# antao97/SegGroup

Hardware: AMD Instinct MI355X
Metric: pseudo-label scenes/sec (150k pts, 1.5k segs) (higher is better)
Workload: dtype f32 (fp32 accumulate; operands split into 2 x fp16 pieces on v_mfma_f32_32x32x16_f16; kNN / FPS scores in exact fp32 order); 1 GPU; 64 distinct synthetic scenes per GPU per step, 150000 pts / 1500 segs each (BASELINE.json configs[2]; configs[1] = the same scene shape, single scene); mode=ins_infer, scenes_in_flight=112, engine=14 groups x 8 scenes per batched launch, weights=tests/golden/weights_g2.npz, parallelism=scene-parallel x1

## Files before the change

### include/seggroup_hip.h

```cpp
#ifndef SEGGROUP_HIP_H
#define SEGGROUP_HIP_H

#include <stddef.h>
#include <stdint.h>

#ifdef __cplusplus
extern "C" {
#endif

#define SG_OK          0
#define SG_EINVAL     -1
#define SG_EHIP       -2
#define SG_ENOMEM     -3
#define SG_ESTALL     -4
#define SG_EUNSUP     -5
#define SG_EINTERNAL  -6

#define SG_MODE_INS_INFER 0
#define SG_MODE_SEM_INFER 1

#define SG_NUM_LABEL_VECTORS 14
#define SG_RANGE_WORDS 256
#define SG_MAX_POINTS (1 << 20)

const char* sg_last_error(void);
int  sg_version(void);
int  sg_device_count(void);
int  sg_selftest_wave_ops(int* h_mismatches, void* stream);
int  sg_selftest_list_insert(int* h_mismatches, void* stream);

size_t sg_contract_ws_bytes(int S);
int sg_contract_point_edges(const int64_t* d_adj, int E, const int32_t* d_seg_of_point, int N, int S,
                            int32_t* d_out_adj, int out_capacity, int32_t* d_out_count,
                            void* d_ws, size_t ws_bytes, void* stream);

int sg_gather_members(const int32_t* d_seg_points, const int32_t* d_seg_off, int S,
                      const int32_t* d_order, const int32_t* d_dst, const int32_t* d_cl,
                      int32_t* d_members, int32_t* d_pos_of_point, int32_t* d_cluster_of_pos,
                      int32_t* d_slot_of_pos, void* stream);

size_t sg_fps_ws_bytes(int N);
int sg_fps_sample(const float* d_data, int N, int ch_in, const int32_t* d_members, const int32_t* d_cl_off, int C,
                  int P, int ch_out, int transform, float* d_samples, int32_t* d_sel,
                  void* d_ws, size_t ws_bytes, void* stream);

size_t sg_mlp1_ws_bytes(int C);
int sg_mlp1_forward(const float* d_samples, int C, const float* d_w, const float* d_gamma, const float* d_beta,
                    float* d_feat, int feat_stride, void* d_ws, size_t ws_bytes, void* stream);

int sg_edge_distance(const float* d_feat, int feat_stride, int D, const int32_t* d_adj, int E,
                     float* d_dist, void* stream);

int sg_group_max_rows(const float* d_rows, int row_stride, int D, const int32_t* d_goff, const int32_t* d_gidx,
                      int G, float* d_out, int out_stride, void* stream);

int sg_segment_max(const float* d_rows, int N, int D, const int32_t* d_cluster_of_pos,
                   float* d_out, int out_stride, int C, void* stream);

size_t sg_center_ws_bytes(int T, int C);
int sg_center_clusters(const float* d_data, int N, const int32_t* d_members, const int32_t* d_cl_off, int C,
                       const int32_t* d_tile_cl, const int32_t* d_tile_lo, const int32_t* d_tile_hi, int T,
                       const int32_t* d_cl_tile_off, float* d_x9m, float* d_xyzw,
                       void* d_ws, size_t ws_bytes, void* stream);

int sg_cluster_knn(const float* d_xyzw, int N, const int32_t* d_cl_off,
                   const int32_t* d_tile_cl, const int32_t* d_tile_lo, const int32_t* d_tile_hi, int T,
                   int k, int pos0, int32_t* d_knn, void* stream);

int sg_segment_boxes(const float* d_data, const int32_t* d_seg_points, const int32_t* d_seg_off, int S,
                     float* d_box, void* stream);
int sg_cluster_knn_pruned(const float* d_xyzw, int N, const int32_t* d_cl_off,
                          const int32_t* d_tile_cl, const int32_t* d_tile_lo, const int32_t* d_tile_hi, int T,
                          const int32_t* d_cl_seg_off, const int32_t* d_order, const int32_t* d_dst,
                          const int32_t* d_seg_off, const float* d_segbox, const int32_t* d_slot_of_pos,
                          int k, int pos0, int32_t* d_knn, void* stream);

size_t sg_segment_sort_ws_bytes(int N);
int sg_segment_sort_boxes(const float* d_data, int N, const int32_t* d_seg_points, const int32_t* d_seg_off,
                          const int32_t* d_seg_of_point, int S, const int32_t* d_seg_chunk_off, int max_seg, float* d_segbox,
                          int32_t* d_sperm, float* d_chunk_box, double* d_seg_sums, void* d_ws, size_t ws_bytes, void* stream);
int sg_layer_layout(const float* d_data, int N, const int32_t* d_seg_points, const int32_t* d_seg_off, const int32_t* d_sperm, int S,
                    const int32_t* d_order, const int32_t* d_dst, const int32_t* d_cl, const float* d_cl_mean, int32_t* d_members,
                    int32_t* d_pos_of_point, int32_t* d_cluster_of_pos, int32_t* d_slot_of_pos, float* d_x9m, float* d_sxyzw,
                    int32_t* d_smpos, float* d_point_rec, int32_t* d_seed_id, unsigned int* d_range_bits, void* stream);
int sg_knn_operands(const float* d_data, const int32_t* d_seg_points, const int32_t* d_seg_off, const int32_t* d_sperm, int S,
                    const int32_t* d_order, const int32_t* d_dst, float* d_sxyzw, int32_t* d_smpos, void* stream);
int sg_cluster_knn_sorted(const float* d_sxyzw, const int32_t* d_smpos, int N, const int32_t* d_cl_off,
                          const int32_t* d_tile_cl, const int32_t* d_tile_lo, const int32_t* d_tile_hi, int T,
                          const int32_t* d_cl_seg_off, const int32_t* d_order, const int32_t* d_dst,
                          const int32_t* d_seg_off, const int32_t* d_seg_chunk_off, const float* d_segbox,
                          const float* d_chunk_box, const int32_t* d_slot_of_pos, int k, int pos0, int32_t* d_knn, void* stream);
int sg_knn_seed_points(const int32_t* d_knn, const int32_t* d_members, int N, int k, int32_t* d_seed, void* stream);
int sg_cluster_knn_seeded(const float* d_sxyzw, const int32_t* d_smpos, int N, const int32_t* d_cl_off,
                          const int32_t* d_tile_cl, const int32_t* d_tile_lo, const int32_t* d_tile_hi, int T,
                          const int32_t* d_cl_seg_off, const int32_t* d_order, const int32_t* d_dst,
                          const int32_t* d_seg_off, const int32_t* d_seg_chunk_off, const float* d_segbox,
                          const float* d_chunk_box, const int32_t* d_slot_of_pos, const int32_t* d_seed,
                          const int32_t* d_seg_prevcl, const int32_t* d_members, const float* d_point_rec,
                          int k, int pos0, int32_t* d_knn, void* stream);

int sg_knn_chunk_table(const int32_t* d_order, const int32_t* d_dst, const int32_t* d_seg_off, const int32_t* d_seg_chunk_off,
                       const float* d_chunk_box, int S, const int32_t* d_slot_chunk0, float* d_cc, void* stream);
int sg_cluster_knn_2pass(const float* d_sxyzw, const int32_t* d_smpos, int N, const int32_t* d_cl_off,
                         const int32_t* d_tile_cl, const int32_t* d_tile_lo, const int32_t* d_tile_hi,
                         const int32_t* d_tile_chunk0, int T, const int32_t* d_cl_chunk_off, const float* d_cc,
                         int k, int pos0, int32_t* d_knn, void* stream);
int sg_cluster_knn_sorted_w(const float* d_sxyzw, const int32_t* d_smpos, int N, const int32_t* d_cl_off,
                            const int32_t* d_tile_cl, const int32_t* d_tile_lo, const int32_t* d_tile_hi, int T,
                            const int32_t* d_cl_seg_off, const int32_t* d_order, const int32_t* d_dst,
                            const int32_t* d_seg_off, const int32_t* d_seg_chunk_off, const float* d_segbox,
                            const float* d_chunk_box, const int32_t* d_slot_of_pos, int k, int pos0, int waves_per_tile,
                            int32_t* d_knn, void* stream);

size_t sg_edgeconv_ws_bytes(int N);
int sg_edgeconv_forward(const float* d_x9m, const int32_t* d_knn, int N, int k, int layers,
                        const float* d_w1, const float* d_g1, const float* d_b1,
                        const float* d_w2, const float* d_g2, const float* d_b2,
                        float* d_out, void* d_ws, size_t ws_bytes, void* stream);
int sg_edgeconv_forward_r(const float* d_x9m, const int32_t* d_knn, int N, int k, int layers, const float* d_w1, const float* d_g1,
                          const float* d_b1, const float* d_w2, const float* d_g2, const float* d_b2, float* d_out, void* d_ws,
                          size_t ws_bytes, unsigned int* d_range_bits, void* stream);
#define SG_EDGECONV_COMPILER_LOOP 1u
int sg_edgeconv_forward_x(const float* d_x9m, const int32_t* d_knn, int N, int k, int layers, const float* d_w1, const float* d_g1,
                          const float* d_b1, const float* d_w2, const float* d_g2, const float* d_b2, float* d_out, void* d_ws,
                          size_t ws_bytes, unsigned int* d_range_bits, unsigned int flags, void* stream);
int sg_edge_range(const float* d_x9m, int N, unsigned int* d_range_bits, void* stream);

size_t sg_gcn_ws_bytes(int S, int D, int E);
int sg_gcn_forward(const float* d_x, int S, int D, const int32_t* d_adj, int E,
                   const int32_t* d_rowptr, const int32_t* d_col, const int32_t* d_eid,
                   const float* d_w, float alpha, float* d_out, void* d_ws, size_t ws_bytes, void* stream);

int sg_export_labels(const int32_t* d_unmap, int V, const int32_t* d_seg_of_point, int N,
                     const int32_t* d_tables, int T, int S, int32_t* d_out, void* stream);

size_t sg_eval_ws_bytes(int max_ins);
int sg_evaluate(const int32_t* d_gt, const int32_t* d_sem_pred, const int32_t* d_ins_pred, int V, int max_ins,
                float* h_iou_sem, float* h_iou_ins, float* h_acc, void* d_ws, size_t ws_bytes, void* stream);

typedef struct sg_partition sg_partition;

sg_partition* sg_partition_create(int S, const int32_t* h_seg_first, const int32_t* h_seg_size,
                                  const int32_t* h_seg_ins, const int32_t* h_seg_sem);
void sg_partition_destroy(sg_partition* p);
int  sg_partition_num_clusters(const sg_partition* p);

int sg_partition_union(sg_partition* p, int seg_root1, int seg_root2);
int sg_partition_find(const sg_partition* p, int s);
int sg_partition_label(const sg_partition* p, int r, int32_t* ins, int32_t* sem, double* npts);

int sg_partition_layer(const sg_partition* p, int32_t* h_root, int32_t* h_cl_of_seg, int32_t* h_order,
                       int32_t* h_cl_seg_off, int32_t* h_cl_pt_off, int32_t* h_dst);

int sg_partition_group_nearby(sg_partition* p, const int32_t* h_root, int C, const float* h_dist,
                              const int32_t* h_adj, int E, float th, uint8_t* h_connected);

int sg_partition_contract(const sg_partition* p, const int32_t* h_root_old, const int32_t* h_adj, int E,
                          const uint8_t* h_keep, int32_t* h_adj_out);

int sg_partition_group_unlabeled(sg_partition* p, int32_t* h_root_io, int* C_io, float* h_feat, int D,
                                 int32_t* h_adj, int* E_io);
int sg_partition_unlabeled_fallback(sg_partition* p, const int32_t* h_root, int C, const float* h_samples, int P);

int sg_partition_export_tables(const sg_partition* p, int32_t* h_seg_tab, int32_t* h_ins_tab, int32_t* h_sem_tab);

typedef struct sg_pipeline sg_pipeline;

typedef struct sg_weights {
    const float* mlp1_w;  const float* mlp1_g;  const float* mlp1_b;
    const float* mlp2_w;  const float* mlp2_g;  const float* mlp2_b;
    const float* gcn2_w;
    const float* mlp3_w1; const float* mlp3_g1; const float* mlp3_b1;
    const float* mlp3_w2; const float* mlp3_g2; const float* mlp3_b2;
    const float* gcn3_w;
} sg_weights;

typedef struct sg_scene {
    int N, S, E0, V;
    const float*   d_data;
    const int64_t* d_adj;
    const int32_t* d_seg_of_point;
    const int32_t* d_seg_points;
    const int32_t* d_seg_off;
    const int32_t* d_unmap;
    const int32_t* d_gt;
    const int32_t* h_seg_first;
    const int32_t* h_seg_size;
    const int32_t* h_seg_ins;
    const int32_t* h_seg_sem;
    const int32_t* h_seg_of_vertex;
} sg_scene;

typedef struct sg_result {
    int32_t* h_labels;
    float iou_sem[80];
    float iou_ins[80];
    float acc[4];
    int32_t trace[5];
    int32_t stalled;
    int32_t used_fallback;
    int32_t* h_tables;
// ... 425 lines not shown
```

### seggroup_amd/csrc/kernels_mlp1.hip

```cpp
#include "engine_ctx.h"
#include "sg_common.h"
#include "knn_device.h"
#include "wave_ops.h"

namespace {

constexpr int K1 = 10;

__device__ inline float knn_score(float xq, float yq, float zq, float xxq, float xc, float yc, float zc, float xxc) {
    const float t = __builtin_fmaf(zq, zc, __builtin_fmaf(yq, yc, xq * xc));
    const float inner = -2.0f * t;
    return ((-xxc) - inner) - xxq;
}

__device__ inline float sqnorm3(float x, float y, float z) { return (x * x + y * y) + z * z; }

__device__ __forceinline__ void mlp1_knn_moments_body(const float* __restrict__ samples, uint8_t* __restrict__ knn,
                                                      double* __restrict__ partial, int c) {
    const int lane = threadIdx.x;
    const float* row = samples + ((size_t)c * 64 + lane) * 6;
    float f[6];
#pragma unroll
    for (int k = 0; k < 6; ++k) f[k] = row[k];
    const float xx = sqnorm3(f[0], f[1], f[2]);

    double kvl[K1];
#pragma unroll
    for (int t = 0; t < K1; ++t) kvl[t] = sgknn::list_empty();
#pragma unroll 8
    for (int j = 0; j < 64; ++j) {
        const float s = knn_score(f[0], f[1], f[2], xx, sgw::bcast(f[0], j), sgw::bcast(f[1], j), sgw::bcast(f[2], j), sgw::bcast(xx, j));
        sgknn::list_insert<K1>(kvl, sgknn::make_key(s, j));
    }
    int bi[K1];
#pragma unroll
    for (int t = 0; t < K1; ++t) bi[t] = sgknn::list_index(kvl[t]);
    uint8_t* ko = knn + ((size_t)c * 64 + lane) * K1;
#pragma unroll
    for (int t = 0; t < K1; ++t) ko[t] = (uint8_t)bi[t];

    double e[K1][6];
    double m0 = 0, m1 = 0, m2 = 0;
#pragma unroll
    for (int t = 0; t < K1; ++t) {
#pragma unroll
        for (int k = 0; k < 6; ++k) e[t][k] = (double)__shfl(f[k], bi[t]);
        m0 += e[t][0]; m1 += e[t][1]; m2 += e[t][2];
    }
    m0 /= K1; m1 /= K1; m2 /= K1;
    double acc[27];
#pragma unroll
    for (int q = 0; q < 27; ++q) acc[q] = 0.0;
#pragma unroll
    for (int t = 0; t < K1; ++t) {
        e[t][0] = (e[t][0] - m0) * 10.0; e[t][1] = (e[t][1] - m1) * 10.0; e[t][2] = (e[t][2] - m2) * 10.0;
        int q = 6;
#pragma unroll
        for (int a = 0; a < 6; ++a) {
            acc[a] += e[t][a];
#pragma unroll
            for (int b = a; b < 6; ++b) acc[q++] += e[t][a] * e[t][b];
        }
    }
#pragma unroll
    for (int q = 0; q < 27; ++q) {
        const double v = sgw::wave_sum(acc[q]);
        if (lane == 0) partial[(size_t)c * 27 + q] = v;
    }
}
__global__ __launch_bounds__(64) void k_mlp1_knn_moments(const float* __restrict__ samples, uint8_t* __restrict__ knn,
                                                         double* __restrict__ partial) {
    mlp1_knn_moments_body(samples, knn, partial, blockIdx.x);
}
__global__ __launch_bounds__(64) void k_mlp1_knn_moments_b(const sg::SlotCtx* __restrict__ cx) {
    const sg::SlotCtx& c = cx[blockIdx.y];
    if ((int)blockIdx.x >= c.S) return;
    mlp1_knn_moments_body(c.samples, c.m1_knn, c.m1_partial, blockIdx.x);
}

__device__ __forceinline__ void mlp1_finalize_body(const double* __restrict__ partial, int C, const float* __restrict__ w,
                                                   const float* __restrict__ gamma, const float* __restrict__ beta,
                                                   float* __restrict__ folded) {
    __shared__ double mom[27];
    {
        const int q = threadIdx.x >> 5, l = threadIdx.x & 31;
        double s = 0.0;
        for (int c = l; c < C; c += 32) s += partial[(size_t)c * 27 + q];
#pragma unroll
        for (int o = 16; o > 0; o >>= 1) s += __shfl_xor(s, o);
        if (l == 0) mom[q] = s / ((double)C * 64.0 * K1);
    }
    __syncthreads();
    const int ch = threadIdx.x;
    if (ch >= 64) return;
    double cov[6][6];
    int q = 6;
    for (int a = 0; a < 6; ++a)
        for (int b = a; b < 6; ++b) { cov[a][b] = cov[b][a] = mom[q] - mom[a] * mom[b]; ++q; }
    double mean = 0.0, var = 0.0;
    for (int a = 0; a < 6; ++a) {
        mean += (double)w[ch * 6 + a] * mom[a];
        for (int b = 0; b < 6; ++b) var += (double)w[ch * 6 + a] * (double)w[ch * 6 + b] * cov[a][b];
    }
    const double a_ = (double)gamma[ch] / sqrt(var + 1e-5);
    for (int k = 0; k < 6; ++k) folded[ch * 6 + k] = (float)(a_ * (double)w[ch * 6 + k]);
    folded[384 + ch] = (float)((double)beta[ch] - a_ * mean);
}
__global__ __launch_bounds__(27 * 32) void k_mlp1_finalize(const double* __restrict__ partial, int C, const float* __restrict__ w,
                                                           const float* __restrict__ gamma, const float* __restrict__ beta,
                                                           float* __restrict__ folded) {
    mlp1_finalize_body(partial, C, w, gamma, beta, folded);
}
__global__ __launch_bounds__(27 * 32) void k_mlp1_finalize_b(const sg::SlotCtx* __restrict__ cx, const float* __restrict__ w,
                                                             const float* __restrict__ gamma, const float* __restrict__ beta) {
    const sg::SlotCtx& c = cx[blockIdx.y];
    mlp1_finalize_body(c.m1_partial, c.S, w, gamma, beta, c.m1_folded);
}

__device__ __forceinline__ void mlp1_apply_body(const float* __restrict__ samples, const uint8_t* __restrict__ knn,
                                                const float* __restrict__ folded, float* __restrict__ feat, int feat_stride, int c) {
    const int lane = threadIdx.x;
    const float* row = samples + ((size_t)c * 64 + lane) * 6;
    float f[6];
#pragma unroll
    for (int k = 0; k < 6; ++k) f[k] = row[k];
    const uint8_t* ki = knn + ((size_t)c * 64 + lane) * K1;
    float e[K1][6];
    double m0 = 0, m1 = 0, m2 = 0;
    double ed[K1][3];
#pragma unroll
    for (int t = 0; t < K1; ++t) {
        const int j = ki[t];
#pragma unroll
        for (int k = 0; k < 6; ++k) e[t][k] = __shfl(f[k], j);
        ed[t][0] = e[t][0]; ed[t][1] = e[t][1]; ed[t][2] = e[t][2];
        m0 += ed[t][0]; m1 += ed[t][1]; m2 += ed[t][2];
    }
    m0 /= K1; m1 /= K1; m2 /= K1;
#pragma unroll
    for (int t = 0; t < K1; ++t) {
        e[t][0] = (float)((ed[t][0] - m0) * 10.0); e[t][1] = (float)((ed[t][1] - m1) * 10.0); e[t][2] = (float)((ed[t][2] - m2) * 10.0);
    }
    float* out = feat + (size_t)c * feat_stride;
    __shared__ float hs[64 * 65];
    __shared__ __attribute__((aligned(8))) float wl[448];
#pragma unroll
    for (int i = 0; i < 7; ++i) {
        const int e_ = lane + 64 * i;
        wl[e_ < 384 ? (e_ % 6) * 64 + e_ / 6 : e_] = folded[e_];
    }
    __builtin_amdgcn_wave_barrier();
    using f32x2 = __attribute__((ext_vector_type(2))) float;
#pragma unroll 2
    for (int ch = 0; ch < 64; ch += 2) {
        f32x2 w[6];
#pragma unroll
        for (int k = 0; k < 6; ++k) w[k] = *reinterpret_cast<const f32x2*>(&wl[k * 64 + ch]);
        const f32x2 b = *reinterpret_cast<const f32x2*>(&wl[384 + ch]);
        float h0 = -INFINITY, h1 = -INFINITY;
#pragma unroll
        for (int t = 0; t < K1; ++t) {
            f32x2 y = b;
#pragma unroll
            for (int k = 0; k < 6; ++k) y = __builtin_elementwise_fma(w[k], f32x2{e[t][k], e[t][k]}, y);
            h0 = fmaxf(h0, y.x);
            h1 = fmaxf(h1, y.y);
        }
        hs[ch * 65 + lane] = fmaxf(h0, 0.2f * h0);
        hs[(ch + 1) * 65 + lane] = fmaxf(h1, 0.2f * h1);
    }
    __builtin_amdgcn_wave_barrier();
    {
        const float* row = hs + lane * 65;
        float mx = -INFINITY;
        double sm = 0.0;
#pragma unroll 8
        for (int i = 0; i < 64; ++i) {
            const float v = row[i];
            mx = fmaxf(mx, v);
            sm += (double)v;
        }
        out[lane] = mx;
        out[64 + lane] = (float)(sm / 64.0);
    }
}
__global__ __launch_bounds__(64) void k_mlp1_apply(const float* __restrict__ samples, const uint8_t* __restrict__ knn,
                                                   const float* __restrict__ folded, float* __restrict__ feat, int feat_stride) {
    mlp1_apply_body(samples, knn, folded, feat, feat_stride, blockIdx.x);
}
__global__ __launch_bounds__(64) void k_mlp1_apply_b(const sg::SlotCtx* __restrict__ cx) {
    const sg::SlotCtx& c = cx[blockIdx.y];
    if ((int)blockIdx.x >= c.S) return;
    mlp1_apply_body(c.samples, c.m1_knn, c.m1_folded, c.feat1, 128, blockIdx.x);
}

__global__ __launch_bounds__(27 * 32) void k_mlp1_bwd_stats(const double* __restrict__ partial, int C, const float* __restrict__ w,
                                                            double* __restrict__ mom_out, float* __restrict__ cst, float* __restrict__ stats_out) {
    __shared__ double mom[27];
    {
        const int q = threadIdx.x >> 5, l = threadIdx.x & 31;
        double s = 0.0;
        for (int c = l; c < C; c += 32) s += partial[(size_t)c * 27 + q];
#pragma unroll
        for (int o = 16; o > 0; o >>= 1) s += __shfl_xor(s, o);
        if (l == 0) { mom[q] = s / ((double)C * 64.0 * K1); mom_out[q] = mom[q]; }
    }
    __syncthreads();
    const int ch = threadIdx.x;
    if (ch >= 64) return;
    double cov[6][6];
    int q = 6;
    for (int a = 0; a < 6; ++a)
        for (int b = a; b < 6; ++b) { cov[a][b] = cov[b][a] = mom[q] - mom[a] * mom[b]; ++q; }
    double mean = 0.0, var = 0.0;
    for (int a = 0; a < 6; ++a) {
        mean += (double)w[ch * 6 + a] * mom[a];
        for (int b = 0; b < 6; ++b) var += (double)w[ch * 6 + a] * (double)w[ch * 6 + b] * cov[a][b];
    }
    var = fmax(var, 0.0);
    cst[ch] = (float)mean;
    cst[64 + ch] = (float)(1.0 / sqrt(var + 1e-5));
    if (stats_out) { stats_out[ch] = (float)mean; stats_out[64 + ch] = (float)var; }
}

__global__ __launch_bounds__(64) void k_mlp1_bwd_rows(const float* __restrict__ samples, const uint8_t* __restrict__ knn, const float* __restrict__ w,
                                                      const float* __restrict__ gamma, const float* __restrict__ beta, const float* __restrict__ cst,
                                                      const float* __restrict__ gfeat, int g_stride, double* __restrict__ rows_partial) {
    const int c = blockIdx.x, lane = threadIdx.x;
    const float* row = samples + ((size_t)c * 64 + lane) * 6;
    float f[6];
#pragma unroll
    for (int k = 0; k < 6; ++k) f[k] = row[k];
    const uint8_t* ki = knn + ((size_t)c * 64 + lane) * K1;
    float e[K1][6];
    double m0 = 0, m1 = 0, m2 = 0;
    double ed[K1][3];
#pragma unroll
    for (int t = 0; t < K1; ++t) {
        const int j = ki[t];
#pragma unroll
        for (int k = 0; k < 6; ++k) e[t][k] = __shfl(f[k], j);
        ed[t][0] = e[t][0]; ed[t][1] = e[t][1]; ed[t][2] = e[t][2];
        m0 += ed[t][0]; m1 += ed[t][1]; m2 += ed[t][2];
    }
    m0 /= K1; m1 /= K1; m2 /= K1;
#pragma unroll
    for (int t = 0; t < K1; ++t) {
        e[t][0] = (float)((ed[t][0] - m0) * 10.0); e[t][1] = (float)((ed[t][1] - m1) * 10.0); e[t][2] = (float)((ed[t][2] - m2) * 10.0);
    }
    const float* g = gfeat + (size_t)c * g_stride;
    double* out = rows_partial + (size_t)c * 512;
    for (int ch = 0; ch < 64; ++ch) {
        const float w0 = w[ch * 6 + 0], w1 = w[ch * 6 + 1], w2 = w[ch * 6 + 2], w3 = w[ch * 6 + 3], w4 = w[ch * 6 + 4], w5 = w[ch * 6 + 5];
        const float mu = cst[ch], inv = cst[64 + ch], ga = gamma[ch], be = beta[ch];
        float best = -INFINITY, bx = 0.f, ba = 0.f;
        float be_[6] = {0.f, 0.f, 0.f, 0.f, 0.f, 0.f};
#pragma unroll
        for (int t = 0; t < K1; ++t) {
            float y = w0 * e[t][0];
            y = __builtin_fmaf(w1, e[t][1], y); y = __builtin_fmaf(w2, e[t][2], y);
            y = __builtin_fmaf(w3, e[t][3], y); y = __builtin_fmaf(w4, e[t][4], y); y = __builtin_fmaf(w5, e[t][5], y);
            const float xh = (y - mu) * inv;
            const float a = xh * ga + be;
            const float h = fmaxf(a, 0.2f * a);
            if (h > best) {
                best = h; bx = xh; ba = a;
#pragma unroll
                for (int k = 0; k < 6; ++k) be_[k] = e[t][k];
            }
        }
        float mv = best;
        int mi = lane;
        sgw::wave_argmax(mv, mi);
        const float dh = (lane == mi ? g[ch] : 0.f) + g[64 + ch] * (1.0f / 64.0f);
        const double da = (double)(dh * (ba > 0.f ? 1.f : 0.2f));
        const double v[8] = {da, da * (double)bx, da * (double)be_[0], da * (double)be_[1], da * (double)be_[2], da * (double)be_[3],
                             da * (double)be_[4], da * (double)be_[5]};
#pragma unroll
        for (int q = 0; q < 8; ++q) {
            const double r = sgw::wave_sum(v[q]);
            if (lane == 0) out[ch * 8 + q] = r;
        }
    }
}

__global__ __launch_bounds__(512) void k_mlp1_bwd_fold(const double* __restrict__ rows_partial, int nparts, int C, const double* __restrict__ mom,
                                                       const float* __restrict__ w, const float* __restrict__ gamma, const float* __restrict__ cst,
                                                       float* __restrict__ gw, float* __restrict__ gg, float* __restrict__ gb) {
    __shared__ double acc[512];
    const int t = threadIdx.x;
    double a = 0.0;
    for (int c = 0; c < nparts; ++c) a += rows_partial[(size_t)c * 512 + t];
    acc[t] = a;
    __syncthreads();
    const double rows = (double)C * 64.0 * K1;
    if (t < 64) { gb[t] = (float)acc[t * 8]; gg[t] = (float)acc[t * 8 + 1]; }
    if (t < 384) {
        const int ch = t / 6, j = t - ch * 6;
        const double inv = (double)cst[64 + ch], mu = (double)cst[ch];
        auto m2 = [&](int p, int q_) {
            const int lo = p < q_ ? p : q_, hi = p < q_ ? q_ : p;
            return mom[6 + lo * 6 - lo * (lo - 1) / 2 + (hi - lo)];
        };
        double wsee = 0.0;
        for (int q_ = 0; q_ < 6; ++q_) wsee += (double)w[ch * 6 + q_] * m2(q_, j);
        const double xe = (wsee - mu * mom[j]) * inv * rows;
        gw[t] = (float)((double)gamma[ch] * inv * (acc[ch * 8 + 2 + j] - acc[ch * 8] / rows * (mom[j] * rows) - acc[ch * 8 + 1] / rows * xe));
    }
}

}

namespace sg {

int b_mlp1(const SlotCtx* d_ctx, const float* d_w, const float* d_g, const float* d_b, const BatchDims& bd, hipStream_t st) {
    if (bd.nslots == 0 || bd.max_S == 0) return SG_OK;
    k_mlp1_knn_moments_b<<<dim3(bd.max_S, bd.nslots), 64, 0, st>>>(d_ctx);
    k_mlp1_finalize_b<<<dim3(1, bd.nslots), 27 * 32, 0, st>>>(d_ctx, d_w, d_g, d_b);
    k_mlp1_apply_b<<<dim3(bd.max_S, bd.nslots), 64, 0, st>>>(d_ctx);
    SG_LAUNCH_CHECK();
    return SG_OK;
}

}

extern "C" {

size_t sg_mlp1_ws_bytes(int C) {
    const size_t c = (size_t)std::max(C, 1);
    return sg::align_up(c * 64 * K1) + sg::align_up(c * 27 * 8) + sg::align_up(448 * 4);
}

int sg_mlp1_forward(const float* d_samples, int C, const float* d_w, const float* d_gamma, const float* d_beta, float* d_feat,
                    int feat_stride, void* d_ws, size_t ws_bytes, void* stream) {
    SG_REQUIRE(C >= 0 && feat_stride >= 128 && d_ws, "sg_mlp1_forward: bad arguments");
    if (C == 0) return SG_OK;
    sg::Carver cv(d_ws, ws_bytes);
    uint8_t* knn = cv.take<uint8_t>((size_t)C * 64 * K1);
    double* partial = cv.take<double>((size_t)C * 27);
    float* folded = cv.take<float>(448);
    if (!cv.ok) return sg::fail(SG_ENOMEM, "sg_mlp1_forward: workspace too small (%zu < %zu)", ws_bytes, sg_mlp1_ws_bytes(C));
    hipStream_t st = sg::as_stream(stream);
    k_mlp1_knn_moments<<<C, 64, 0, st>>>(d_samples, knn, partial);
    k_mlp1_finalize<<<1, 27 * 32, 0, st>>>(partial, C, d_w, d_gamma, d_beta, folded);
    k_mlp1_apply<<<C, 64, 0, st>>>(d_samples, knn, folded, d_feat, feat_stride);
    SG_LAUNCH_CHECK();
    return SG_OK;
}

size_t sg_mlp1_backward_ws_bytes(int C) {
    const size_t c = (size_t)std::max(C, 1);
    return sg::align_up(c * 64 * K1) + sg::align_up(c * 27 * 8) + sg::align_up(c * 512 * 8) + sg::align_up(27 * 8) + sg::align_up(128 * 4) + sg::align_up(512 * 8);
}

int sg_mlp1_backward(const float* d_samples, int C, const float* d_w, const float* d_gamma, const float* d_beta, const float* d_gfeat,
                     int g_stride, float* d_gw, float* d_gg, float* d_gb, float* d_bn_stats, void* d_ws, size_t ws_bytes, void* stream) {
    SG_REQUIRE(C > 0 && g_stride >= 128 && d_samples && d_w && d_gamma && d_beta && d_gfeat && d_gw && d_gg && d_gb && d_ws, "sg_mlp1_backward: bad arguments");
    sg::Carver cv(d_ws, ws_bytes);
    uint8_t* knn = cv.take<uint8_t>((size_t)C * 64 * K1);
    double* partial = cv.take<double>((size_t)C * 27);
    double* rows_partial = cv.take<double>((size_t)C * 512);
    double* mom = cv.take<double>(27);
    float* cst = cv.take<float>(128);
    double* red = cv.take<double>(512);
    if (!cv.ok) return sg::fail(SG_ENOMEM, "sg_mlp1_backward: workspace too small (%zu < %zu)", ws_bytes, sg_mlp1_backward_ws_bytes(C));
    hipStream_t st = sg::as_stream(stream);
    k_mlp1_knn_moments<<<C, 64, 0, st>>>(d_samples, knn, partial);
    k_mlp1_bwd_stats<<<1, 27 * 32, 0, st>>>(partial, C, d_w, mom, cst, d_bn_stats);
    k_mlp1_bwd_rows<<<C, 64, 0, st>>>(d_samples, knn, d_w, d_gamma, d_beta, cst, d_gfeat, g_stride, rows_partial);
    if (int rc = sg::reduce_partials(rows_partial, C, 512, 512, red, st)) return rc;
    k_mlp1_bwd_fold<<<1, 512, 0, st>>>(red, 1, C, mom, d_w, d_gamma, cst, d_gw, d_gg, d_gb);
    SG_LAUNCH_CHECK();
    return SG_OK;
}

}
```

### seggroup_amd/hip.py

```python
from __future__ import annotations

import contextlib
import ctypes as C
import os
import struct
import types
from typing import Optional

_HERE = os.path.dirname(os.path.abspath(__file__))
LIB_PATH = os.environ.get("SEGGROUP_HIP_LIB") or os.path.join(_HERE, "libseggroup_hip.so")
HOST_LIB_OVERRIDE = os.environ.get("SEGGROUP_HIP_HOST_LIB")

SG_OK, SG_EINVAL, SG_EHIP, SG_ENOMEM, SG_ESTALL, SG_EUNSUP, SG_EINTERNAL = 0, -1, -2, -3, -4, -5, -6
MODE_INS_INFER, MODE_SEM_INFER = 0, 1
COLOUR_SEMANTIC, COLOUR_INSTANCE, COLOUR_SEGMENT, COLOUR_GROUPING = 0, 1, 2, 3
NUM_LABEL_VECTORS = 14
KNN_BRUTE, KNN_GRID = 0, 1
KNN_INDEX = {"brute": KNN_BRUTE, "grid": KNN_GRID}
MAX_GRID_POINTS = 1 << 24
MAX_POINTS = 1 << 20
MAX_CLOUD_POINTS = 1 << 27
MAX_RADIUS_PAIRS = 1 << 30


def knn_index(index) -> int:
    if not isinstance(index, str) or index not in KNN_INDEX:
        raise ValueError("index must be 'brute' or 'grid', not %r" % (index,))
    return KNN_INDEX[index]


def knn_cell(cell) -> float:
    c = 0.0 if cell is None else float(cell)
    if not (c >= 0.0) or c == float("inf"):
        raise ValueError("cell must be a finite edge > 0, or None for the library's choice")
    return c
LABEL_NAMES = [f"layer_{l}.{k}" for l in (1, 2, 3, 4) for k in ("seg", "ins", "sem")] + ["final.ins", "final.sem"]

c_f32p = C.POINTER(C.c_float)
c_i32p = C.POINTER(C.c_int32)
c_i64p = C.POINTER(C.c_int64)
c_u8p = C.POINTER(C.c_uint8)
vp = C.c_void_p


class SgError(RuntimeError):
    def __init__(self, code: int, msg: str):
        super().__init__(f"libseggroup_hip error {code}: {msg}")
        self.code = code


class Weights(C.Structure):
    _fields_ = [(n, vp) for n in ("mlp1_w", "mlp1_g", "mlp1_b", "mlp2_w", "mlp2_g", "mlp2_b", "gcn2_w",
                                  "mlp3_w1", "mlp3_g1", "mlp3_b1", "mlp3_w2", "mlp3_g2", "mlp3_b2", "gcn3_w")]


class Scene(C.Structure):
    _fields_ = [("N", C.c_int), ("S", C.c_int), ("E0", C.c_int), ("V", C.c_int),
                ("d_data", vp), ("d_adj", vp), ("d_seg_of_point", vp), ("d_seg_points", vp), ("d_seg_off", vp),
                ("d_unmap", vp), ("d_gt", vp),
                ("h_seg_first", vp), ("h_seg_size", vp), ("h_seg_ins", vp), ("h_seg_sem", vp), ("h_seg_of_vertex", vp)]


class Result(C.Structure):
    _fields_ = [("h_labels", vp), ("iou_sem", C.c_float * 80), ("iou_ins", C.c_float * 80), ("acc", C.c_float * 4),
                ("trace", C.c_int32 * 5), ("stalled", C.c_int32), ("used_fallback", C.c_int32), ("h_tables", vp)]


class Classifier(C.Structure):
    _fields_ = [(n, vp) for n in ("w1", "gamma", "beta", "w2", "b2")]


class Debug(C.Structure):
    _fields_ = [("d_samples1", vp), ("d_feat1", vp), ("d_pointfeat", vp * 2), ("d_knn", vp * 2), ("d_members", vp * 2),
                ("h_gcn", vp * 2), ("h_dist", vp * 3), ("h_adj", vp * 4), ("n_adj", C.c_int32 * 4),
                ("h_feat5", vp), ("h_ins5", vp), ("h_sem5", vp), ("n5", C.c_int32), ("tape", vp), ("d_cat", vp * 2)]


_I, _Z = C.c_int, C.c_size_t
SIGNATURES = {
    "sg_last_error": (C.c_char_p, []),
    "sg_version": (_I, []),
    "sg_device_count": (_I, []),
    "sg_selftest_wave_ops": (_I, [C.POINTER(C.c_int), vp]),
    "sg_selftest_list_insert": (_I, [C.POINTER(C.c_int), vp]),
    "sg_contract_ws_bytes": (_Z, [_I]),
    "sg_contract_point_edges": (_I, [vp, _I, vp, _I, _I, vp, _I, vp, vp, _Z, vp]),
    "sg_gather_members": (_I, [vp, vp, _I, vp, vp, vp, vp, vp, vp, vp, vp]),
    "sg_fps_ws_bytes": (_Z, [_I]),
    "sg_fps_sample": (_I, [vp, _I, _I, vp, vp, _I, _I, _I, _I, vp, vp, vp, _Z, vp]),
    "sg_mlp1_ws_bytes": (_Z, [_I]),
    "sg_mlp1_forward": (_I, [vp, _I, vp, vp, vp, vp, _I, vp, _Z, vp]),
    "sg_edge_distance": (_I, [vp, _I, _I, vp, _I, vp, vp]),
    "sg_group_max_rows": (_I, [vp, _I, _I, vp, vp, _I, vp, _I, vp]),
    "sg_segment_max": (_I, [vp, _I, _I, vp, vp, _I, _I, vp]),
    "sg_center_ws_bytes": (_Z, [_I, _I]),
    "sg_center_clusters": (_I, [vp, _I, vp, vp, _I, vp, vp, vp, _I, vp, vp, vp, vp, _Z, vp]),
    "sg_cluster_knn": (_I, [vp, _I, vp, vp, vp, vp, _I, _I, _I, vp, vp]),
    "sg_segment_boxes": (_I, [vp, vp, vp, _I, vp, vp]),
    "sg_cluster_knn_pruned": (_I, [vp, _I, vp, vp, vp, vp, _I, vp, vp, vp, vp, vp, vp, _I, _I, vp, vp]),
    "sg_segment_sort_ws_bytes": (_Z, [_I]),
    "sg_knn_operands": (_I, [vp, vp, vp, vp, _I, vp, vp, vp, vp, vp]),
    "sg_cluster_knn_sorted": (_I, [vp, vp, _I, vp, vp, vp, vp, _I, vp, vp, vp, vp, vp, vp, vp, vp, _I, _I, vp, vp]),
    "sg_segment_sort_boxes": (_I, [vp, _I, vp, vp, vp, _I, vp, _I, vp, vp, vp, vp, vp, _Z, vp]),
    "sg_layer_layout": (_I, [vp, _I, vp, vp, vp, _I, vp, vp, vp, vp, vp, vp, vp, vp, vp, vp, vp, vp, vp, vp, vp]),
    "sg_cluster_knn_sorted_w": (_I, [vp, vp, _I, vp, vp, vp, vp, _I, vp, vp, vp, vp, vp, vp, vp, vp, _I, _I, _I, vp, vp]),
    "sg_knn_seed_points": (_I, [vp, vp, _I, _I, vp, vp]),
    "sg_cluster_knn_seeded": (_I, [vp, vp, _I, vp, vp, vp, vp, _I, vp, vp, vp, vp, vp, vp, vp, vp, vp, vp, vp, vp, _I, _I, vp, vp]),
    "sg_knn_chunk_table": (_I, [vp, vp, vp, vp, vp, _I, vp, vp, vp]),
    "sg_cluster_knn_2pass": (_I, [vp, vp, _I, vp, vp, vp, vp, vp, _I, vp, vp, _I, _I, vp, vp]),
    "sg_nearest_point_ws_bytes": (_Z, [_I]),
    "sg_nearest_point": (_I, [vp, _I, vp, _I, _I, vp, vp, _Z, vp]),
    "sg_prep_sample_ws_bytes": (_Z, [_I, _I]),
    "sg_prep_sample_points": (_I, [vp, vp, _I, vp, _I, vp, vp, C.POINTER(C.c_int), vp, _Z, vp]),
    "sg_pointcloud_adjacency_ws_bytes": (_Z, [_I, _I]),
    "sg_pointcloud_adjacency": (_I, [vp, _I, _I, _I, vp, C.POINTER(C.c_int), vp, _Z, vp]),
    "sg_mesh_adjacency_ws_bytes": (_Z, [_I]),
    "sg_mesh_adjacency": (_I, [vp, _I, vp, _I, vp, C.POINTER(C.c_int), vp, C.POINTER(C.c_int), vp, _Z, vp]),
    "sg_segment_lists_ws_bytes": (_Z, [_I, _I]),
    "sg_segment_lists": (_I, [vp, _I, vp, _I, vp, vp, vp, C.POINTER(C.c_int), vp, _Z, vp]),
    "sg_write_seg_json": (_I, [C.c_char_p, vp, vp, _I, _I]),
    "sg_overseg_ws_bytes": (_Z, [_I, _I]),
    "sg_overseg_edges": (_I, [vp, _I, vp, _I, vp, vp, vp, vp, C.POINTER(C.c_int), vp, _Z, vp]),
    "sg_overseg_merge": (_I, [vp, vp, _I, _I, C.c_float, _I, vp]),
    "sg_overseg_scan": (_I, [vp, _I, vp, _I, C.c_float, _I, vp, vp, _Z, vp]),
    "sg_overseg_set_timing": (_I, [_I]),
    "sg_overseg_stage_times": (_I, [vp, _I]),
    "sg_overseg_stage_name": (C.c_char_p, [_I]),
    "sg_write_segs_json": (_I, [C.c_char_p, C.c_char_p, vp, _I, C.c_float, _I]),
    "sg_pointcloud_knn_ws_bytes": (_Z, [_I]),
    "sg_pointcloud_knn": (_I, [vp, _I, _I, _I, vp, vp, _Z, vp]),
    "sg_pointcloud_normals": (_I, [vp, _I, vp, _I, vp, vp, vp, _Z, vp]),
    "sg_pcseg_ws_bytes": (_Z, [_I, _I]),
    "sg_pcseg_edges": (_I, [vp, _I, _I, vp, vp, vp, vp, vp, C.POINTER(C.c_int), vp, _Z, vp]),
    "sg_pcseg_scan": (_I, [vp, _I, _I, vp, C.c_float, _I, vp, vp, _Z, vp]),
    "sg_pcseg_set_timing": (_I, [_I]),
    "sg_pcseg_stage_times": (_I, [vp, _I]),
    "sg_pcseg_stage_name": (C.c_char_p, [_I]),
    "sg_cloud_thin_ws_bytes": (_Z, [_I]),
    "sg_cloud_thin": (_I, [vp, _I, _I, C.c_float, vp, vp, C.POINTER(C.c_int), vp, vp, _Z, vp]),
    "sg_cloud_thin_set_timing": (_I, [_I]),
    "sg_cloud_thin_stage_times": (_I, [vp, _I]),
    "sg_cloud_thin_stage_name": (C.c_char_p, [_I]),
    "sg_pointcloud_knn_grid_ws_bytes": (_Z, [_I, _I]),
    "sg_pointcloud_knn_grid": (_I, [vp, _I, _I, _I, C.c_float, vp, vp, _Z, vp]),
    "sg_pointcloud_knn_grid_set_timing": (_I, [_I]),
    "sg_pointcloud_knn_grid_stage_times": (_I, [vp, _I]),
    "sg_pointcloud_knn_grid_stage_name": (C.c_char_p, [_I]),
    "sg_pointcloud_knn_grid_stats": (_I, [vp, _I]),
    "sg_pointcloud_knn_grid_set_tuning": (_I, [_I, _I]),
    "sg_pcseg_ws_bytes_indexed": (_Z, [_I, _I, _I]),
    "sg_pcseg_edges_indexed": (_I, [vp, _I, _I, vp, _I, C.c_float, vp, vp, vp, vp, C.POINTER(C.c_int), vp, _Z, vp]),
    "sg_pcseg_scan_indexed": (_I, [vp, _I, _I, vp, _I, C.c_float, C.c_float, _I, vp, vp, _Z, vp]),
    "sg_nearest_point_grid_ws_bytes": (_Z, [_I, _I]),
    "sg_nearest_point_grid": (_I, [vp, _I, _I, vp, _I, _I, C.c_float, vp, vp, vp, _Z, vp]),
    "sg_nearest_point_grid_set_timing": (_I, [_I]),
    "sg_nearest_point_grid_stage_times": (_I, [vp, _I]),
    "sg_nearest_point_grid_stage_name": (C.c_char_p, [_I]),
    "sg_nearest_point_grid_stats": (_I, [vp, _I]),
    "sg_nearest_point_grid_set_tuning": (_I, [_I, _I]),
    "sg_cloud_knn_cross_grid_ws_bytes": (_Z, [_I, _I, _I]),
    "sg_cloud_knn_cross_grid": (_I, [vp, _I, _I, vp, _I, _I, _I, C.c_float, vp, vp, vp, _Z, vp]),
    "sg_cloud_knn_cross_grid_set_timing": (_I, [_I]),
    "sg_cloud_knn_cross_grid_stage_times": (_I, [vp, _I]),
    "sg_cloud_knn_cross_grid_stage_name": (C.c_char_p, [_I]),
    "sg_cloud_knn_cross_grid_stats": (_I, [vp, _I]),
    "sg_cloud_knn_cross_grid_set_tuning": (_I, [_I, _I]),
    "sg_knn_vote": (_I, [vp, _I, _I, vp, _I, vp, vp, vp, vp, vp]),
    "sg_rigid_apply": (_I, [vp, _I, _I, vp, vp, vp]),
    "sg_align_moments_ws_bytes": (_Z, [_I]),
    "sg_align_moments": (_I, [vp, _I, _I, vp, _I, _I, vp, vp, C.c_float, vp, vp, vp, vp, _Z, vp]),
    "sg_align_solve": (_I, [vp, vp, vp, vp]),
    "sg_align_plane_moments_ws_bytes": (_Z, [_I]),
    "sg_align_plane_moments": (_I, [vp, _I, _I, vp, vp, _I, _I, vp, _I, vp, vp, C.c_float, vp, vp, vp, _Z, vp]),
    "sg_align_plane_solve": (_I, [vp, vp, C.c_double, vp, vp, vp]),
    "sg_fpfh_ws_bytes": (_Z, [_I]),
    "sg_fpfh": (_I, [vp, _I, _I, vp, vp, vp, vp, vp, vp, _Z, vp]),
    "sg_feature_nearest": (_I, [vp, _I, vp, _I, _I, vp, vp, vp]),
    "sg_ransac_ws_bytes": (_Z, [_I, _I]),
    "sg_ransac_count": (_I, [vp, _I, _I, vp, _I, _I, vp, vp, _I, _I, C.c_uint64, vp, C.c_double, C.c_double, C.c_double, vp, C.POINTER(C.c_int),
                             vp, _Z, vp]),
    "sg_ransac_set_tuning": (_I, [_I, _I]),
    "sg_ransac_stage_times": (_I, [vp, _I]),
    "sg_ransac_stage_name": (C.c_char_p, [_I]),
    "sg_triangle_pose": (_I, [vp, vp, vp]),
    "sg_plane_ransac_ws_bytes": (_Z, [_I, _I, _I]),
    "sg_plane_ransac": (_I, [vp, _I, _I, vp, vp, C.c_double, _I, C.c_uint64, vp, C.c_double, C.c_double, C.c_double, vp, vp, C.POINTER(C.c_int),
                             C.POINTER(C.c_int), vp, _Z, vp]),
    "sg_plane_moments_ws_bytes": (_Z, [_I]),
    "sg_plane_moments": (_I, [vp, _I, _I, vp, vp, C.c_double, vp, C.c_double, vp, vp, vp, _Z, vp]),
    "sg_plane_fit": (_I, [vp, vp, vp, vp, vp]),
    "sg_plane_assign_ws_bytes": (_Z, [_I]),
    "sg_plane_assign": (_I, [vp, _I, _I, vp, C.c_double, vp, C.c_double, _I, vp, C.POINTER(C.c_int), vp, _Z, vp]),
    "sg_plane_set_tuning": (_I, [_I, _I]),
    "sg_plane_stage_times": (_I, [vp, _I]),
    "sg_plane_stage_name": (C.c_char_p, [_I]),
    "sg_label_index_ws_bytes": (_Z, [_I]),
    "sg_label_index": (_I, [vp, _I, vp, vp, vp, C.POINTER(C.c_int), C.POINTER(C.c_int), vp, _Z, vp]),
    "sg_label_moments_ws_bytes": (_Z, [_I, _I]),
    "sg_label_moments": (_I, [vp, _I, _I, vp, vp, _I, vp, vp, vp, vp, _Z, vp]),
    "sg_label_yaw_boxes_ws_bytes": (_Z, [_I, _I, _I]),
    "sg_label_yaw_boxes": (_I, [vp, _I, _I, vp, vp, _I, vp, _I, vp, vp, vp, vp, _Z, vp]),
    "sg_label_frame_extents_ws_bytes": (_Z, [_I, _I]),
    "sg_label_frame_extents": (_I, [vp, _I, _I, vp, vp, _I, vp, vp, vp, _Z, vp]),
    "sg_box_axes": (_I, [vp, vp, vp]),
    "sg_label_set_tuning": (_I, [_I]),
    "sg_label_stage_times": (_I, [vp, _I]),
    "sg_label_stage_name": (C.c_char_p, [_I]),
    "sg_components_ws_bytes": (_Z, [_I]),
    "sg_components_edges": (_I, [vp, C.c_longlong, _I, vp, vp, vp, C.POINTER(C.c_int), vp, _Z, vp]),
    "sg_components_faces": (_I, [vp, _I, _I, vp, vp, vp, C.POINTER(C.c_int), vp, _Z, vp]),
    "sg_components_knn": (_I, [vp, _I, vp, _I, _I, C.c_float, vp, vp, vp, C.POINTER(C.c_int), vp, _Z, vp]),
    "sg_components_set_timing": (_I, [_I]),
    "sg_components_stage_times": (_I, [vp, _I]),
    "sg_components_stage_name": (C.c_char_p, [_I]),
    "sg_radius_grid_ws_bytes": (_Z, [_I]),
    "sg_radius_count_grid": (_I, [vp, _I, _I, C.c_float, C.c_float, vp, vp, _Z, vp]),
    "sg_components_radius": (_I, [vp, _I, _I, C.c_float, C.c_float, vp, vp, vp, C.POINTER(C.c_int), vp, _Z, vp]),
    "sg_radius_grid_set_timing": (_I, [_I]),
    "sg_radius_grid_stage_times": (_I, [vp, _I]),
    "sg_radius_grid_stage_name": (C.c_char_p, [_I]),
    "sg_radius_grid_stats": (_I, [vp, _I]),
    "sg_radius_neighbours_ws_bytes": (_Z, [_I, C.c_int64]),
    "sg_radius_neighbours_grid": (_I, [vp, _I, _I, C.c_float, C.c_float, C.c_int64, vp, vp, C.POINTER(C.c_int64), vp, _Z, vp]),
    "sg_pointcloud_normals_csr": (_I, [vp, _I, vp, vp, vp, vp, vp, _Z, vp]),
    "sg_pcseg_ws_bytes_radius": (_Z, [_I, C.c_int64]),
    "sg_pcseg_edges_radius": (_I, [vp, _I, C.c_float, C.c_float, C.c_int64, vp, vp, vp, vp, vp, vp, C.POINTER(C.c_int), C.POINTER(C.c_int64),
                                   vp, _Z, vp]),
    "sg_pcseg_scan_radius": (_I, [vp, _I, C.c_float, C.c_float, C.c_int64, vp, C.c_float, _I, vp, C.POINTER(C.c_int64), vp, _Z, vp]),
    "sg_pcseg_radius_set_timing": (_I, [_I]),
    "sg_pcseg_radius_stage_times": (_I, [vp, _I]),
    "sg_pcseg_radius_stage_name": (C.c_char_p, [_I]),
    "sg_segment_vote_ws_bytes": (_Z, [_I]),
    "sg_segment_rank": (_I, [vp, _I, vp, vp, vp, C.POINTER(C.c_int), vp, _Z, vp]),
    "sg_segment_vote": (_I, [vp, vp, _I, _I] + [vp] * 9 + [C.POINTER(C.c_int), vp, _Z, vp]),
    "sg_segment_vote_set_timing": (_I, [_I]),
    "sg_segment_vote_stage_times": (_I, [vp, _I]),
    "sg_segment_vote_stage_name": (C.c_char_p, [_I]),
    "sg_rekey_clicks": (_I, [vp, vp, _I, vp, vp, vp, _I, vp, _I, vp, vp, _I, vp, vp, vp]),
    "sg_segment_graph_ws_bytes": (_Z, [C.c_longlong, _I]),
    "sg_segment_graph": (_I, [vp, C.c_longlong, vp, _I, _I, vp, vp, C.POINTER(C.c_longlong), vp, _Z, vp]),
    "sg_segment_graph_set_timing": (_I, [_I]),
    "sg_segment_graph_stage_times": (_I, [vp, _I]),
    "sg_segment_graph_stage_name": (C.c_char_p, [_I]),
    "sg_click_clusters": (_I, [vp, C.c_longlong, vp, _I, vp, vp, vp, C.POINTER(C.c_int)]),
# ... 254 lines not shown
```

Before: 3518 scenes/s.

## Compute MLP1 edge conv with fp32 MFMA 32x32x2 instead of VALU FMAs

Result: no change. 3529 scenes/s (median of 6 runs) (+0.3%).

```diff
diff --git a/include/seggroup_hip.h b/include/seggroup_hip.h
--- a/include/seggroup_hip.h
+++ b/include/seggroup_hip.h
@@ -47,6 +47,11 @@
 size_t sg_mlp1_ws_bytes(int C);
 int sg_mlp1_forward(const float* d_samples, int C, const float* d_w, const float* d_gamma, const float* d_beta,
                     float* d_feat, int feat_stride, void* d_ws, size_t ws_bytes, void* stream);
+#define SG_MLP1_APPLY_DEFAULT 0
+#define SG_MLP1_APPLY_MFMA 1
+#define SG_MLP1_APPLY_VALU 2
+int sg_mlp1_forward_v(const float* d_samples, int C, const float* d_w, const float* d_gamma, const float* d_beta,
+                      float* d_feat, int feat_stride, int variant, void* d_ws, size_t ws_bytes, void* stream);
 
 int sg_edge_distance(const float* d_feat, int feat_stride, int D, const int32_t* d_adj, int E,
                      float* d_dist, void* stream);
diff --git a/seggroup_amd/csrc/kernels_mlp1.hip b/seggroup_amd/csrc/kernels_mlp1.hip
--- a/seggroup_amd/csrc/kernels_mlp1.hip
+++ b/seggroup_amd/csrc/kernels_mlp1.hip
@@ -1,3 +1,6 @@
+#include <cstdlib>
+#include <cstring>
+
 #include "engine_ctx.h"
 #include "sg_common.h"
 #include "knn_device.h"
@@ -117,15 +120,13 @@
     mlp1_finalize_body(c.m1_partial, c.S, w, gamma, beta, c.m1_folded);
 }
 
-__device__ __forceinline__ void mlp1_apply_body(const float* __restrict__ samples, const uint8_t* __restrict__ knn,
-                                                const float* __restrict__ folded, float* __restrict__ feat, int feat_stride, int c) {
+__device__ __forceinline__ void mlp1_edge_rows(const float* __restrict__ samples, const uint8_t* __restrict__ knn, int c, float (&e)[K1][6]) {
     const int lane = threadIdx.x;
     const float* row = samples + ((size_t)c * 64 + lane) * 6;
     float f[6];
 #pragma unroll
     for (int k = 0; k < 6; ++k) f[k] = row[k];
     const uint8_t* ki = knn + ((size_t)c * 64 + lane) * K1;
-    float e[K1][6];
     double m0 = 0, m1 = 0, m2 = 0;
     double ed[K1][3];
 #pragma unroll
@@ -141,15 +142,42 @@
     for (int t = 0; t < K1; ++t) {
         e[t][0] = (float)((ed[t][0] - m0) * 10.0); e[t][1] = (float)((ed[t][1] - m1) * 10.0); e[t][2] = (float)((ed[t][2] - m2) * 10.0);
     }
-    float* out = feat + (size_t)c * feat_stride;
-    __shared__ float hs[64 * 65];
-    __shared__ __attribute__((aligned(8))) float wl[448];
+}
+
+__device__ __forceinline__ void mlp1_stage_folded(const float* __restrict__ folded, float* __restrict__ wl) {
+    const int lane = threadIdx.x;
 #pragma unroll
     for (int i = 0; i < 7; ++i) {
         const int e_ = lane + 64 * i;
         wl[e_ < 384 ? (e_ % 6) * 64 + e_ / 6 : e_] = folded[e_];
     }
     __builtin_amdgcn_wave_barrier();
+}
+
+__device__ __forceinline__ void mlp1_reduce_samples(const float* __restrict__ hs, float* __restrict__ out) {
+    const int lane = threadIdx.x;
+    __builtin_amdgcn_wave_barrier();
+    const float* row = hs + lane * 65;
+    float mx = -INFINITY;
+    double sm = 0.0;
+#pragma unroll 8
+    for (int i = 0; i < 64; ++i) {
+        const float v = row[i];
+        mx = fmaxf(mx, v);
+        sm += (double)v;
+    }
+    out[lane] = mx;
+    out[64 + lane] = (float)(sm / 64.0);
+}
+
+__device__ __forceinline__ void mlp1_apply_valu_body(const float* __restrict__ samples, const uint8_t* __restrict__ knn,
+                                                     const float* __restrict__ folded, float* __restrict__ feat, int feat_stride, int c) {
+    const int lane = threadIdx.x;
+    float e[K1][6];
+    mlp1_edge_rows(samples, knn, c, e);
+    __shared__ float hs[64 * 65];
+    __shared__ __attribute__((aligned(8))) float wl[448];
+    mlp1_stage_folded(folded, wl);
     using f32x2 = __attribute__((ext_vector_type(2))) float;
 #pragma unroll 2
     for (int ch = 0; ch < 64; ch += 2) {
@@ -169,30 +197,92 @@
         hs[ch * 65 + lane] = fmaxf(h0, 0.2f * h0);
         hs[(ch + 1) * 65 + lane] = fmaxf(h1, 0.2f * h1);
     }
-    __builtin_amdgcn_wave_barrier();
-    {
-        const float* row = hs + lane * 65;
-        float mx = -INFINITY;
-        double sm = 0.0;
-#pragma unroll 8
-        for (int i = 0; i < 64; ++i) {
-            const float v = row[i];
-            mx = fmaxf(mx, v);
-            sm += (double)v;
-        }
-        out[lane] = mx;
-        out[64 + lane] = (float)(sm / 64.0);
-    }
-}
-__global__ __launch_bounds__(64) void k_mlp1_apply(const float* __restrict__ samples, const uint8_t* __restrict__ knn,
+    mlp1_reduce_samples(hs, feat + (size_t)c * feat_stride);
+}
+
+__device__ __forceinline__ void mlp1_apply_mfma_body(const float* __restrict__ samples, const uint8_t* __restrict__ knn,
+                                                     const float* __restrict__ folded, float* __restrict__ feat, int feat_stride, int c) {
+    const int lane = threadIdx.x, l32 = lane & 31, hi = lane >> 5;
+    float e[K1][6];
+    mlp1_edge_rows(samples, knn, c, e);
+    __shared__ float hs[64 * 65];
+    __shared__ __attribute__((aligned(16))) float wl[448];
+    mlp1_stage_folded(folded, wl);
+    using f32x4 = __attribute__((ext_vector_type(4))) float;
+    using f32x16 = __attribute__((ext_vector_type(16))) float;
+    float a[2][3];
+    f32x16 sh[2];
+#pragma unroll
+    for (int ct = 0; ct < 2; ++ct) {
+#pragma unroll
+        for (int s = 0; s < 3; ++s) a[ct][s] = wl[(2 * s + hi) * 64 + 32 * ct + l32];
+#pragma unroll
+        for (int q = 0; q < 4; ++q) {
+            const f32x4 v = *reinterpret_cast<const f32x4*>(&wl[384 + 32 * ct + 8 * q + 4 * hi]);
+            sh[ct][4 * q] = v.x; sh[ct][4 * q + 1] = v.y; sh[ct][4 * q + 2] = v.z; sh[ct][4 * q + 3] = v.w;
+        }
+    }
+#pragma unroll
+    for (int t = 0; t < K1; ++t) {
+#pragma unroll
+        for (int s = 0; s < 3; ++s) {
+            const auto r = __builtin_amdgcn_permlane32_swap(__float_as_uint(e[t][2 * s]), __float_as_uint(e[t][2 * s + 1]), false, false);
+            e[t][2 * s] = __uint_as_float(r[0]);
+            e[t][2 * s + 1] = __uint_as_float(r[1]);
+        }
+    }
+#pragma unroll
+    for (int half = 0; half < 2; ++half) {
+        f32x16 h[2];
+#pragma unroll
+        for (int ct = 0; ct < 2; ++ct)
+#pragma unroll
+            for (int r = 0; r < 16; ++r) h[ct][r] = -INFINITY;
+#pragma unroll
+        for (int t = 0; t < K1; ++t) {
+#pragma unroll
+            for (int ct = 0; ct < 2; ++ct) {
+                f32x16 y = sh[ct];
+#pragma unroll
+                for (int s = 0; s < 3; ++s) y = __builtin_amdgcn_mfma_f32_32x32x2f32(a[ct][s], e[t][2 * s + half], y, 0, 0, 0);
+#pragma unroll
+                for (int r = 0; r < 16; ++r) h[ct][r] = fmaxf(h[ct][r], y[r]);
+            }
+        }
+#pragma unroll
+        for (int ct = 0; ct < 2; ++ct)
+#pragma unroll
+            for (int r = 0; r < 16; ++r) {
+                const int ch = 32 * ct + 8 * (r >> 2) + 4 * hi + (r & 3);
+                hs[ch * 65 + 32 * half + l32] = fmaxf(h[ct][r], 0.2f * h[ct][r]);
+            }
+    }
+    mlp1_reduce_samples(hs, feat + (size_t)c * feat_stride);
+}
+
+__global__ __launch_bounds__(64, 2) void k_mlp1_apply(const float* __restrict__ samples, const uint8_t* __restrict__ knn,
                                                    const float* __restrict__ folded, float* __restrict__ feat, int feat_stride) {
-    mlp1_apply_body(samples, knn, folded, feat, feat_stride, blockIdx.x);
-}
-__global__ __launch_bounds__(64) void k_mlp1_apply_b(const sg::SlotCtx* __restrict__ cx) {
+    mlp1_apply_mfma_body(samples, knn, folded, feat, feat_stride, blockIdx.x);
+}
+__global__ __launch_bounds__(64, 2) void k_mlp1_apply_b(const sg::SlotCtx* __restrict__ cx) {
     const sg::SlotCtx& c = cx[blockIdx.y];
     if ((int)blockIdx.x >= c.S) return;
-    mlp1_apply_body(c.samples, c.m1_knn, c.m1_folded, c.feat1, 128, blockIdx.x);
-}
+    mlp1_apply_mfma_body(c.samples, c.m1_knn, c.m1_folded, c.feat1, 128, blockIdx.x);
+}
+__global__ __launch_bounds__(64) void k_mlp1_apply_valu(const float* __restrict__ samples, const uint8_t* __restrict__ knn,
+                                                        const float* __restrict__ folded, float* __restrict__ feat, int feat_stride) {
+    mlp1_apply_valu_body(samples, knn, folded, feat, feat_stride, blockIdx.x);
+}
+__global__ __launch_bounds__(64) void k_mlp1_apply_valu_b(const sg::SlotCtx* __restrict__ cx) {
+    const sg::SlotCtx& c = cx[blockIdx.y];
+    if ((int)blockIdx.x >= c.S) return;
+    mlp1_apply_valu_body(c.samples, c.m1_knn, c.m1_folded, c.feat1, 128, blockIdx.x);
+}
+
+const int g_apply_default = [] {
+    const char* v = getenv("SG_MLP1_APPLY");
+    return v && !strcmp(v, "valu") ? SG_MLP1_APPLY_VALU : SG_MLP1_APPLY_MFMA;
+}();
 
 __global__ __launch_bounds__(27 * 32) void k_mlp1_bwd_stats(const double* __restrict__ partial, int C, const float* __restrict__ w,
                                                             double* __restrict__ mom_out, float* __restrict__ cst, float* __restrict__ stats_out) {
@@ -317,7 +407,8 @@
     if (bd.nslots == 0 || bd.max_S == 0) return SG_OK;
     k_mlp1_knn_moments_b<<<dim3(bd.max_S, bd.nslots), 64, 0, st>>>(d_ctx);
     k_mlp1_finalize_b<<<dim3(1, bd.nslots), 27 * 32, 0, st>>>(d_ctx, d_w, d_g, d_b);
-    k_mlp1_apply_b<<<dim3(bd.max_S, bd.nslots), 64, 0, st>>>(d_ctx);
+    if (g_apply_default == SG_MLP1_APPLY_VALU) k_mlp1_apply_valu_b<<<dim3(bd.max_S, bd.nslots), 64, 0, st>>>(d_ctx);
+    else k_mlp1_apply_b<<<dim3(bd.max_S, bd.nslots), 64, 0, st>>>(d_ctx);
     SG_LAUNCH_CHECK();
     return SG_OK;
 }
@@ -333,7 +424,14 @@
 
 int sg_mlp1_forward(const float* d_samples, int C, const float* d_w, const float* d_gamma, const float* d_beta, float* d_feat,
                     int feat_stride, void* d_ws, size_t ws_bytes, void* stream) {
+    return sg_mlp1_forward_v(d_samples, C, d_w, d_gamma, d_beta, d_feat, feat_stride, SG_MLP1_APPLY_DEFAULT, d_ws, ws_bytes, stream);
+}
+
+int sg_mlp1_forward_v(const float* d_samples, int C, const float* d_w, const float* d_gamma, const float* d_beta, float* d_feat,
+                      int feat_stride, int variant, void* d_ws, size_t ws_bytes, void* stream) {
     SG_REQUIRE(C >= 0 && feat_stride >= 128 && d_ws, "sg_mlp1_forward: bad arguments");
+    SG_REQUIRE(variant == SG_MLP1_APPLY_DEFAULT || variant == SG_MLP1_APPLY_MFMA || variant == SG_MLP1_APPLY_VALU, "sg_mlp1_forward_v: unknown variant");
+    if (variant == SG_MLP1_APPLY_DEFAULT) variant = g_apply_default;
     if (C == 0) return SG_OK;
     sg::Carver cv(d_ws, ws_bytes);
     uint8_t* knn = cv.take<uint8_t>((size_t)C * 64 * K1);
@@ -343,7 +441,8 @@
     hipStream_t st = sg::as_stream(stream);
     k_mlp1_knn_moments<<<C, 64, 0, st>>>(d_samples, knn, partial);
     k_mlp1_finalize<<<1, 27 * 32, 0, st>>>(partial, C, d_w, d_gamma, d_beta, folded);
-    k_mlp1_apply<<<C, 64, 0, st>>>(d_samples, knn, folded, d_feat, feat_stride);
+    if (variant == SG_MLP1_APPLY_VALU) k_mlp1_apply_valu<<<C, 64, 0, st>>>(d_samples, knn, folded, d_feat, feat_stride);
+    else k_mlp1_apply<<<C, 64, 0, st>>>(d_samples, knn, folded, d_feat, feat_stride);
     SG_LAUNCH_CHECK();
     return SG_OK;
 }
diff --git a/seggroup_amd/hip.py b/seggroup_amd/hip.py
--- a/seggroup_amd/hip.py
+++ b/seggroup_amd/hip.py
@@ -90,6 +90,7 @@
     "sg_fps_sample": (_I, [vp, _I, _I, vp, vp, _I, _I, _I, _I, vp, vp, vp, _Z, vp]),
     "sg_mlp1_ws_bytes": (_Z, [_I]),
     "sg_mlp1_forward": (_I, [vp, _I, vp, vp, vp, vp, _I, vp, _Z, vp]),
+    "sg_mlp1_forward_v": (_I, [vp, _I, vp, vp, vp, vp, _I, _I, vp, _Z, vp]),
     "sg_edge_distance": (_I, [vp, _I, _I, vp, _I, vp, vp]),
     "sg_group_max_rows": (_I, [vp, _I, _I, vp, vp, _I, vp, _I, vp]),
     "sg_segment_max": (_I, [vp, _I, _I, vp, vp, _I, _I, vp]),
```
